# xiph/vorbis

Hardware: NVIDIA H100
Metric: stereo_blocks_per_sec_mdct_psy (higher is better)
Workload: dtype f32

## Files before the change

vorbis_b200/csrc/vb200.cu:

```cuda
#include <cuda_runtime.h>
#include <algorithm>
#include <atomic>
#include <cstdio>
#include <cstdlib>
#include <cstring>
#include <mutex>
#include <string>
#include <type_traits>
#include <vector>

#include "vorbis_b200.h"
#include "vb200_tables.h"
#include "vb200_kernels.cuh"
#include "vb200_cqn.cuh"
#include "vb200_psy2.cuh"
#include "vb200_psy3.cuh"
#include "vb200_floor1.cuh"
#include "vb200_env.cuh"
#include "vb200_res.cuh"
#include "vb200_streams.cuh"
#include "vb200_managed.cuh"
#include "floor1_db_table.h"

using namespace vb200;
// ... 1115 lines not shown
      case 1024: LAUNCH_XF(1024); break;
      case 2048: LAUNCH_XF(2048); break;
      default: LAUNCH_XF(0); break;
    }
#undef LAUNCH_XF
    rc = post_launch(c); if (rc) return rc;
  }
  return 0;
}

static int phaseA_psy_launch(vb200_ctx *c, int W, int nblocks, const vb200_phaseA_io *io, cudaStream_t st,
                             float *d_logfft, float *d_lmax, float *d_gmax) {
  const XformDev &X = c->dx[W];
  const int ch = c->setup.channels, N = X.N;
  const int rows = nblocks * ch;
  int rc;
  {
    const PsyDev &P0 = c->dpsy[2 * W], &P1 = c->dpsy[2 * W + 1];
    const size_t smem = psy2_smem(P0, P1);
    int rc = set_smem(k_phaseA_psy, smem); if (rc) return rc;
    {
      int &tuned = c->psy_carveout_ctas;
      const char *e = getenv("VB200_PSY_CTAS");
      const int ctas = e ? atoi(e) : c->psy_ctas_per_sm;
      if (tuned != ctas) {
        int pct = (int)((ctas * (smem + 1024) * 100 + 228 * 1024 - 1) / (228 * 1024));
        if (pct > 100) pct = 100;
        CU(cudaFuncSetAttribute(k_phaseA_psy, cudaFuncAttributePreferredSharedMemoryCarveout, pct));
        tuned = ctas;
      }
      c->psy_ctas_per_sm = ctas;
    }
    PhaseA2Args A;
    A.mdct_in = io->tap_mdct_raw ? io->tap_mdct_raw : io->mdct;
    A.logfft = d_logfft; A.lmax = d_lmax; A.gmax = d_gmax; A.desc = io->desc;
    A.mdct_out = io->mdct; A.logmdct = io->logmdct; A.logmask = io->logmask; A.ampmax_out = io->ampmax_out;
    A.tap_noise = io->tap_noise; A.tap_tone = io->tap_tone;
    { const char *e = getenv("VB200_DEBUG_SKIP"); A.dbg_skip = e ? atoi(e) : 0; }
    A.dbg_cycles = nullptr;
    if (getenv("VB200_PHASE_TIMING")) {
      void *p; if ((rc = ensure(c, 10, 16 * sizeof(unsigned long long), &p))) return rc;
      A.dbg_cycles = (unsigned long long *)p;
    }
    const int n = N / 2;
    const char *ev = getenv("VB200_PSY_V1");
    const bool v2ok = !(ev && atoi(ev)) && (n == 128 || n == 256 || n == 512 || n == 1024 || n == 2048);
    const char *ev2 = getenv("VB200_PSY_V2");
    const bool v3ok = v2ok && !(ev2 && atoi(ev2)) && P0.linesper == P1.linesper &&
                      psy3_supported(n, P0.total > P1.total ? P0.total : P1.total, P0.linesper);
    if (v3ok) {
      const int total = P0.total > P1.total ? P0.total : P1.total;
      const int nruns = P0.nruns > P1.nruns ? P0.nruns : P1.nruns;
      const int ngrp = P0.ngrp > P1.ngrp ? P0.ngrp : P1.ngrp;
      int R = 1;
      { const char *e = getenv("VB200_PSY_ROWS"); if (e) R = atoi(e) == 1 ? 1 : 2; }
      const size_t row_bytes = sizeof(float) * ((psy3_floats(n, total, nruns, ngrp) + 3) & ~(size_t)3);
      const size_t smem3 = row_bytes * R;
      int ctas = (int)((227 * 1024) / (smem3 + 1024));
      if (ctas > PSY3_MINB / R) ctas = PSY3_MINB / R;
      if (ctas < 1) ctas = 1;
      { const char *e = getenv("VB200_PSY_CTAS"); if (e) ctas = atoi(e); }
      const bool dbg3 = A.dbg_cycles || A.tap_noise || A.tap_tone;
#define LAUNCH_PSY3D(KK, RR, DD)                                                                   \
      do {                                                                                         \
        if ((rc = set_smem(k_phaseA_psy3<KK, RR, DD>, smem3))) return rc;                          \
        k_phaseA_psy3<KK, RR, DD><<<grid_for(c, (rows + RR - 1) / RR, ctas), PSY3_THREADS * RR, smem3, st>>>(P0, P1, ch, rows, A); \
      } while (0)
#define LAUNCH_PSY3R(KK, RR) do { if (dbg3) LAUNCH_PSY3D(KK, RR, true); else LAUNCH_PSY3D(KK, RR, false); } while (0)
#define LAUNCH_PSY4(KK)                                                                            \
      do {                                                                                         \
        if ((rc = set_smem(k_phaseA_psy4<KK>, row_bytes))) return rc;                              \
        k_phaseA_psy4<KK><<<grid_for(c, rows, PSY3_MINB), PSY3_THREADS, row_bytes, st>>>(P0, P1, ch, rows, A); \
      } while (0)
      static const bool psy_v4 = []() { const char *e = getenv("VB200_PSY_V4"); return e && atoi(e); }();
#define LAUNCH_PSY3(KK) do { if (psy_v4) LAUNCH_PSY4(KK); else if (R == 1) LAUNCH_PSY3R(KK, 1); else LAUNCH_PSY3R(KK, 2); } while (0)
      switch (n / 128) {
        case 1: LAUNCH_PSY3(1); break;
        case 2: LAUNCH_PSY3(2); break;
        case 4: LAUNCH_PSY3(4); break;
        case 8: LAUNCH_PSY3(8); break;
        default: LAUNCH_PSY3(16); break;
      }
#undef LAUNCH_PSY3R
#undef LAUNCH_PSY3D
#undef LAUNCH_PSY4
#undef LAUNCH_PSY3
    } else if (v2ok) {
      const int total = P0.total > P1.total ? P0.total : P1.total;
      const int nruns = P0.nruns > P1.nruns ? P0.nruns : P1.nruns;
      const int ngrp = P0.ngrp > P1.ngrp ? P0.ngrp : P1.ngrp;
      const size_t smem2 = sizeof(float) * psy2_floats(n, total, nruns, ngrp);
      int ctas = (int)((227 * 1024) / (smem2 + 1024));
      if (ctas > PSY2_MINB) ctas = PSY2_MINB;
      if (ctas < 1) ctas = 1;
      { const char *e = getenv("VB200_PSY_CTAS"); if (e) ctas = atoi(e); }
#define LAUNCH_PSY2(KK)                                                                            \
      do {                                                                                         \
        if ((rc = set_smem(k_phaseA_psy2<KK>, smem2))) return rc;                                  \
        k_phaseA_psy2<KK><<<grid_for(c, rows, ctas), PSY2_THREADS, smem2, st>>>(P0, P1, ch, rows, A); \
      } while (0)
      switch (n / 128) {
        case 1: LAUNCH_PSY2(1); break;
        case 2: LAUNCH_PSY2(2); break;
        case 4: LAUNCH_PSY2(4); break;
        case 8: LAUNCH_PSY2(8); break;
        default: LAUNCH_PSY2(16); break;
      }
#undef LAUNCH_PSY2
    } else {
      k_phaseA_psy<<<grid_for(c, rows, c->psy_ctas_per_sm), PSY_THREADS, smem, st>>>(P0, P1, ch, rows, A);
    }
    rc = post_launch(c); if (rc) return rc;
  }
  return 0;
}

static int phaseA_launch(vb200_ctx *c, int W, int nblocks, const vb200_phaseA_io *io,
                         int nstreams, int bps, const float *d_amp0, cudaStream_t st,
                         float *d_logfft, float *d_lmax, float *d_gmax, const PcmSrc *pcmsrc = nullptr) {
  PcmSrc psrc;
  if (pcmsrc) psrc = *pcmsrc;
  else { psrc.base = io->pcm; psrc.fmt = 0; psrc.bps = 1; psrc.hop = 0; psrc.stride = 0; psrc.blk_src = nullptr; }
  const XformDev &X = c->dx[W];
  const int ch = c->setup.channels, N = X.N;
  int rc;
  if (c->profiling) CU(cudaEventRecord(c->ev[0], st));
  if ((rc = phaseA_transform_launch(c, W, nblocks, io, psrc, st, d_logfft, d_lmax))) return rc;
  if (c->profiling) CU(cudaEventRecord(c->ev[1], st));
  {
    const int n = N / 2;
    const float secs = (float)n / (float)c->setup.rate;
    const float secs_att = secs * c->setup.ampmax_att_per_sec;
    if (nstreams > 0)
      k_ampmax<<<(nstreams + 127) / 128, 128, 0, st>>>(1, nstreams, bps, ch, io->desc, d_lmax, d_amp0, secs_att, d_gmax);
    else
      k_ampmax<<<(nblocks + 127) / 128, 128, 0, st>>>(0, nblocks, 0, ch, io->desc, d_lmax, nullptr, secs_att, d_gmax);
    int rc = post_launch(c); if (rc) return rc;
  }
// ... 1139 lines not shown
```

vorbis_b200/csrc/vb200_kernels.cuh:

```cuda
#pragma once
#include <cuda_runtime.h>
#include <stdint.h>
#include "vorbis_b200.h"

namespace vb200 {

#define VB_C1 .92387953251128675613F
#define VB_C2 .70710678118654752441F
#define VB_C3 .38268343236508977175F
#define VB_NEGINF (-9999.f)

struct XformDev {
  int N, log2n, nst, nf;
  int fac[8];
  int stage_off[8];
  float scale;
  const float  *trig;
  const int    *bitrev;
  const float2 *stage_tw;
  const float  *win;
  const float  *wa;
};

struct WinDev {
// ... 25 lines not shown
  const int *cls_off;
  int max_cls_len;
};

__device__ __forceinline__ float todB_dev(float x) {
  const unsigned int u = __float_as_uint(x) & 0x7fffffffu;
  return __uint2float_rn(u) * 7.17711438e-7f - 764.6161886f;
}
__device__ __forceinline__ float add345(float x) {
  return (float)((double)x + .345);
}

#ifndef VB200_EMU
__device__ __forceinline__ unsigned smem_u32(const void *p) { return (unsigned)__cvta_generic_to_shared(p); }
__device__ __forceinline__ float lds_f32(unsigned a) { float v; asm volatile("ld.shared.f32 %0, [%1];" : "=f"(v) : "r"(a)); return v; }
__device__ __forceinline__ int lds_s32(unsigned a) { int v; asm volatile("ld.shared.s32 %0, [%1];" : "=r"(v) : "r"(a)); return v; }
__device__ __forceinline__ int lds_s16(unsigned a) { short v; asm volatile("ld.shared.s16 %0, [%1];" : "=h"(v) : "r"(a)); return (int)v; }
__device__ __forceinline__ int4 lds_v4(unsigned a) { int4 v; asm volatile("ld.shared.v4.s32 {%0,%1,%2,%3}, [%4];" : "=r"(v.x), "=r"(v.y), "=r"(v.z), "=r"(v.w) : "r"(a)); return v; }
__device__ __forceinline__ float4 lds_f4(unsigned a) { float4 v; asm volatile("ld.shared.v4.f32 {%0,%1,%2,%3}, [%4];" : "=f"(v.x), "=f"(v.y), "=f"(v.z), "=f"(v.w) : "r"(a)); return v; }
__device__ __forceinline__ void sts_f4(unsigned a, float4 v) { asm volatile("st.shared.v4.f32 [%0], {%1,%2,%3,%4};" :: "r"(a), "f"(v.x), "f"(v.y), "f"(v.z), "f"(v.w) : "memory"); }
__device__ __forceinline__ void sts_s16(unsigned a, int v) { asm volatile("st.shared.s16 [%0], %1;" :: "r"(a), "h"((short)v) : "memory"); }
__device__ __forceinline__ void sts_f32(unsigned a, float v) { asm volatile("st.shared.f32 [%0], %1;" :: "r"(a), "f"(v) : "memory"); }
__device__ __forceinline__ void sts_s32(unsigned a, int v) { asm volatile("st.shared.s32 [%0], %1;" :: "r"(a), "r"(v) : "memory"); }
__device__ __forceinline__ void named_bar_sync(int barid, int nt) { asm volatile("bar.sync %0, %1;" :: "r"(barid), "r"(nt) : "memory"); }
__device__ __forceinline__ float lds_f32_if(unsigned a, float old, bool p) {
  asm volatile("{\n\t.reg .pred q;\n\tsetp.ne.b32 q, %2, 0;\n\t@q ld.shared.f32 %0, [%1];\n\t}" : "+f"(old) : "r"(a), "r"((int)p));
  return old;
}
__device__ __forceinline__ int lds_s16_if(unsigned a, int old, bool p) {
  short v = (short)old;
  asm volatile("{\n\t.reg .pred q;\n\tsetp.ne.b32 q, %2, 0;\n\t@q ld.shared.s16 %0, [%1];\n\t}" : "+h"(v) : "r"(a), "r"((int)p));
  return (int)v;
}
__device__ __forceinline__ int lds_s32_if(unsigned a, int old, bool p) {
  asm volatile("{\n\t.reg .pred q;\n\tsetp.ne.b32 q, %2, 0;\n\t@q ld.shared.s32 %0, [%1];\n\t}" : "+r"(old) : "r"(a), "r"((int)p));
  return old;
}
__device__ __forceinline__ void sts_s32_if(unsigned a, int v, bool p) {
  asm volatile("{\n\t.reg .pred q;\n\tsetp.ne.b32 q, %2, 0;\n\t@q st.shared.s32 [%0], %1;\n\t}" :: "r"(a), "r"(v), "r"((int)p) : "memory");
}
__device__ __forceinline__ void sts_f32_if(unsigned a, float v, bool p) {
  asm volatile("{\n\t.reg .pred q;\n\tsetp.ne.b32 q, %2, 0;\n\t@q st.shared.f32 [%0], %1;\n\t}" :: "r"(a), "f"(v), "r"((int)p) : "memory");
}
__device__ __forceinline__ void sts_s16_if(unsigned a, int v, bool p) {
  asm volatile("{\n\t.reg .pred q;\n\tsetp.ne.b32 q, %2, 0;\n\t@q st.shared.s16 [%0], %1;\n\t}" :: "r"(a), "h"((short)v), "r"((int)p) : "memory");
}
__device__ __forceinline__ void cp_async16(unsigned dst, const void *src) {
  asm volatile("cp.async.cg.shared.global [%0], [%1], 16;" :: "r"(dst), "l"(src) : "memory");
}
__device__ __forceinline__ void cp_async_commit() { asm volatile("cp.async.commit_group;" ::: "memory"); }
__device__ __forceinline__ void cp_async_wait_all() { asm volatile("cp.async.wait_group 0;" ::: "memory"); }
__device__ __forceinline__ void sts_release(unsigned a, int v) { asm volatile("st.release.cta.shared.s32 [%0], %1;" :: "r"(a), "r"(v) : "memory"); }
__device__ __forceinline__ int lds_acquire(unsigned a) { int v; asm volatile("ld.acquire.cta.shared.s32 %0, [%1];" : "=r"(v) : "r"(a) : "memory"); return v; }
__device__ __forceinline__ int lds_volatile(unsigned a) { int v; asm volatile("ld.volatile.shared.s32 %0, [%1];" : "=r"(v) : "r"(a) : "memory"); return v; }
__device__ __forceinline__ void fence_cta() { asm volatile("fence.acq_rel.cta;" ::: "memory"); }
__device__ __forceinline__ void spin_pause(unsigned ns) { __nanosleep(ns); }
__device__ __forceinline__ void prefetch_l2(const void *p) { asm volatile("prefetch.global.L2 [%0];" :: "l"(p)); }
__device__ __forceinline__ void mbar_init1(unsigned a) { asm volatile("mbarrier.init.shared::cta.b64 [%0], 1;" :: "r"(a) : "memory"); }
__device__ __forceinline__ void mbar_arrive_release(unsigned a) {
  asm volatile("{\n\t.reg .b64 st;\n\tmbarrier.arrive.relaxed.cta.shared::cta.b64 st, [%0];\n\t}" :: "r"(a) : "memory");
}
__device__ __forceinline__ void mbar_park(unsigned a, unsigned parity) {
  asm volatile("{\n\t.reg .pred p;\n\tmbarrier.try_wait.parity.acquire.cta.shared::cta.b64 p, [%0], %1;\n\t}" :: "r"(a), "r"(parity) : "memory");
}
#else
__device__ __forceinline__ unsigned smem_u32(const void *p) { return (unsigned)((const unsigned char *)p - cuemu::dyn_smem()); }
__device__ __forceinline__ float lds_f32(unsigned a) { return *reinterpret_cast<const float *>(cuemu::dyn_smem() + a); }
__device__ __forceinline__ int lds_s32(unsigned a) { return *reinterpret_cast<const int *>(cuemu::dyn_smem() + a); }
__device__ __forceinline__ int lds_s16(unsigned a) { return (int)*reinterpret_cast<const short *>(cuemu::dyn_smem() + a); }
__device__ __forceinline__ int4 lds_v4(unsigned a) { return *reinterpret_cast<const int4 *>(cuemu::dyn_smem() + a); }
__device__ __forceinline__ float4 lds_f4(unsigned a) { return *reinterpret_cast<const float4 *>(cuemu::dyn_smem() + a); }
__device__ __forceinline__ void sts_f4(unsigned a, float4 v) { *reinterpret_cast<float4 *>(cuemu::dyn_smem() + a) = v; }
__device__ __forceinline__ void sts_s16(unsigned a, int v) { *reinterpret_cast<short *>(cuemu::dyn_smem() + a) = (short)v; }
__device__ __forceinline__ void sts_f32(unsigned a, float v) { *reinterpret_cast<float *>(cuemu::dyn_smem() + a) = v; }
__device__ __forceinline__ void sts_s32(unsigned a, int v) { *reinterpret_cast<int *>(cuemu::dyn_smem() + a) = v; }
__device__ __forceinline__ void named_bar_sync(int barid, int nt) { cuemu_named_barrier(barid, nt); }
__device__ __forceinline__ void sts_release(unsigned a, int v) { __atomic_store_n(reinterpret_cast<int *>(cuemu::dyn_smem() + a), v, __ATOMIC_RELEASE); }
__device__ __forceinline__ int lds_acquire(unsigned a) { return __atomic_load_n(reinterpret_cast<int *>(cuemu::dyn_smem() + a), __ATOMIC_ACQUIRE); }
__device__ __forceinline__ int lds_volatile(unsigned a) { return __atomic_load_n(reinterpret_cast<int *>(cuemu::dyn_smem() + a), __ATOMIC_ACQUIRE); }
__device__ __forceinline__ void fence_cta() { __atomic_thread_fence(__ATOMIC_ACQ_REL); }
__device__ __forceinline__ void spin_pause(unsigned) { sched_yield(); }
__device__ __forceinline__ void prefetch_l2(const void *) {}
__device__ __forceinline__ void mbar_init1(unsigned) {}
__device__ __forceinline__ void mbar_arrive_release(unsigned) { __atomic_thread_fence(__ATOMIC_RELEASE); }
__device__ __forceinline__ void mbar_park(unsigned, unsigned) { sched_yield(); }
__device__ __forceinline__ void cp_async16(unsigned dst, const void *src) { memcpy(cuemu::dyn_smem() + dst, src, 16); }
__device__ __forceinline__ void cp_async_commit() {}
__device__ __forceinline__ void cp_async_wait_all() {}
__device__ __forceinline__ float lds_f32_if(unsigned a, float old, bool p) { return p ? lds_f32(a) : old; }
__device__ __forceinline__ int lds_s16_if(unsigned a, int old, bool p) { return p ? lds_s16(a) : old; }
__device__ __forceinline__ void sts_f32_if(unsigned a, float v, bool p) { if (p) sts_f32(a, v); }
__device__ __forceinline__ int lds_s32_if(unsigned a, int old, bool p) { return p ? lds_s32(a) : old; }
__device__ __forceinline__ void sts_s32_if(unsigned a, int v, bool p) { if (p) sts_s32(a, v); }
__device__ __forceinline__ void sts_s16_if(unsigned a, int v, bool p) { if (p) sts_s16(a, v); }
#endif

__device__ __forceinline__ float warp_max(float v) {
#pragma unroll
  for (int o = 16; o > 0; o >>= 1) v = fmaxf(v, __shfl_xor_sync(0xffffffffu, v, o));
  return v;
}


template <int NC> struct XLog2 { static constexpr int v = 1 + XLog2<NC / 2>::v; };
template <> struct XLog2<1> { static constexpr int v = 0; };
template <> struct XLog2<0> { static constexpr int v = 0; };

__device__ __forceinline__ int fly_pad(int a) { return a + 2 * (a >> 5) + 2 * (a >> 9); }

__device__ __forceinline__ void dev_fly8(const float4 v0, const float4 v1, float4 &o0, float4 &o1) {
  const float s62 = v1.z + v0.z, d62 = v1.z - v0.z;
  const float s40 = v1.x + v0.x, d40 = v1.x - v0.x;
  const float d51 = v1.y - v0.y, d73 = v1.w - v0.w;
  const float s51 = v1.y + v0.y, s73 = v1.w + v0.w;
  o1.z = s62 + s40;  o1.x = s62 - s40;
  o0.x = d62 + d51;  o0.z = d62 - d51;
  o0.w = d73 + d40;  o0.y = d73 - d40;
  o1.w = s73 + s51;  o1.y = s73 - s51;
}

template <int NC>
__device__ __forceinline__ void dev_butterflies(const XformDev &X, float *x, int tid, int nt, float *padbuf = nullptr) {
  const int N = NC ? NC : X.N;
  const int log2n = NC ? XLog2<NC>::v : X.log2n;
  const int nst = log2n - 6;
  const int n2 = N >> 1;
  const int items = n2 >> 2;
#pragma unroll
  for (int s = 0; s < nst; s++) {
    const int P = n2 >> s;
    const int lq = P >> 2;
    const int sh = log2n - 3 - s;
    const float2 *tw = X.stage_tw + X.stage_off[s];
    for (int u = tid; u < items; u += nt) {
      const int blk = u >> sh, q = u & (lq - 1);
      float *xb = x + P * blk;
      const int a = P - 2 - 2 * q, b = (P >> 1) - 2 - 2 * q;
      const float2 t = __ldg(tw + q);
// ... 808 lines not shown
```

vorbis_b200/csrc/vb200_psy3.cuh:

```cuda
#pragma once
#include "vb200_psy2.cuh"

namespace vb200 {

constexpr int PSY3_THREADS = 128;
constexpr int PSY3_L = 8;
constexpr int PSY3_RB = 7;
#ifndef PSY3_MINB
#define PSY3_MINB 8
#endif

__host__ __device__ inline bool psy3_supported(int n, int total, int linesper) {
  return linesper == PSY3_L && total <= PSY3_THREADS * PSY3_RB && total >= 2 * PSY3_L &&
         (n == 128 || n == 256 || n == 512 || n == 1024 || n == 2048);
}

__host__ __device__ inline size_t psy3_tone_floats(int n, int total, int nruns) {
  const int tp = (total + 7) & ~7, rp = (nruns + 3) & ~3;
  size_t a0 = 4 * (size_t)tp;
  if (a0 < (size_t)n) a0 = n;
  return a0 + 4 * (size_t)rp;
}
__host__ __device__ inline size_t psy3_floats(int n, int total, int nruns, int ngrp) {
  const size_t tone = psy3_tone_floats(n, total, nruns);
// ... 244 lines not shown
}

struct MixOut { float logmask, m, nz, tn; };
__device__ __noinline__ MixOut final_mix_val(float p2, float L, float p1, float noff, float ath, float gmin,
                                             const float *__restrict__ compand, MixConst C, float m) {
  MixOut o;
  const float work = L - p1;
  const float base = L - work;
  int dB = (int)((double)p2 + .5);
  if (dB >= VB200_COMPAND_LEVELS) dB = VB200_COMPAND_LEVELS - 1;
  if (dB < 0) dB = 0;
  const float nz = base + __ldg(compand + dB);
  float tn = ath + C.att;
  if (tn < gmin) tn = gmin;
  o.nz = nz; o.tn = tn;
  float val = nz + noff;
  if (val > C.noisemaxsupp) val = C.noisemaxsupp;
  const float t = tn + C.toneatt;
  o.logmask = val < t ? t : val;
  const float coeffi = -17.2f;
  float de;
  val = val - L;
  if (val > coeffi) {
    de = (float)(1.0 - ((double)(val - coeffi) * 0.005 * (double)C.m_val));
    if (de < 0.f) de = 0.0001f;
  } else {
    de = (float)(1.0 - ((double)(val - coeffi) * 0.0003 * (double)C.m_val));
  }
  o.m = m * de;
  return o;
}

template <int K, int R, bool DBG>
__global__ void __launch_bounds__(PSY3_THREADS * R, PSY3_MINB / R)
k_phaseA_psy3(PsyDev P0, PsyDev P1, int ch, int nrows, PhaseA2Args A) {
  extern __shared__ __align__(16) float sm_cta[];
  constexpr int nt = PSY3_THREADS;
  const int n = K * nt, ns = n + 4, tid = threadIdx.x & (nt - 1), half = threadIdx.x >> 7, lane = tid & 31;
  const int total = P0.total > P1.total ? P0.total : P1.total;
  const int nruns = P0.nruns > P1.nruns ? P0.nruns : P1.nruns;
  const int ngrp = P0.ngrp > P1.ngrp ? P0.ngrp : P1.ngrp;
  const int tp = (total + 7) & ~7;
  const size_t row_floats = (psy3_floats(n, total, nruns, ngrp) + 3) & ~(size_t)3;
  float *sm = sm_cta + half * row_floats;
  float *S = sm;
  float *s_fft = sm;
  float *copies = sm;
  size_t a0 = 4 * (size_t)tp; if (a0 < (size_t)n) a0 = n;
  int4 *run_rec = reinterpret_cast<int4 *>(sm + a0);
  const size_t area = psy3_floats(n, total, nruns, ngrp) - (size_t)((ngrp + 1 + 3) & ~3) - 16;
  float *grp_min = sm + area;
  int *s_misc = reinterpret_cast<int *>(grp_min + ((ngrp + 1 + 3) & ~3));
  for (int row0 = blockIdx.x * R; row0 < nrows; row0 += gridDim.x * R) {
    const int row = row0 + half < nrows ? row0 + half : nrows - 1;
    const int blk = row / ch;
    const PsyDev &P = A.desc[blk].blocktype ? P1 : P0;
    const float *gm = A.mdct_in + (size_t)row * n;
    const float *lf = A.logfft + (size_t)row * n;
    const float g = A.gmax[blk], lmax = A.lmax[row];
    const float att = tone_att(P, lmax);
    float L[K], M[K], p1[K];
    long long tmark = (DBG && A.dbg_cycles) ? clock64() : 0;
    int tph = 0;
#define PHASE_MARK()                                                              \
    do {                                                                          \
      if (DBG && A.dbg_cycles && threadIdx.x == 0) {                                     \
        const long long tnow = clock64();                                         \
        atomicAdd(A.dbg_cycles + tph, (unsigned long long)(tnow - tmark));        \
        tmark = tnow;                                                             \
      }                                                                           \
      tph++;                                                                      \
    } while (0)
#pragma unroll
    for (int k = 0; k < K; k++) {
      const int i = tid + k * nt;
      M[k] = __ldcs(gm + i);
      s_fft[i] = __ldcs(lf + i);
    }
#pragma unroll
    for (int k = 0; k < K; k++) {
      L[k] = add345(todB_dev(M[k]));
      __stcs(A.logmdct + (size_t)row * n + tid + k * nt, L[k]);
    }
#ifndef VB200_NO_PREFETCH
    {
      const int nrow = row0 + gridDim.x * R + half;
      if (nrow < nrows && tid < 2 * (n / 32)) {
        const float *src = tid < n / 32 ? A.mdct_in : A.logfft;
        prefetch_l2(src + (size_t)nrow * n + (tid & (n / 32 - 1)) * 32);
      }
    }
#endif
    __syncthreads();
    PHASE_MARK();
    dev_tone_runs3(P, s_fft, g, att, run_rec, tid);
    __syncthreads();
    PHASE_MARK();
    dev_tone_scatter3(P, copies, tp, run_rec, tid);
    __syncthreads();
    PHASE_MARK();
    dev_chase3<DBG>(P, copies, tp, s_misc, tid, half == 0 ? A.dbg_cycles : nullptr);
    PHASE_MARK();
    const float *seed = copies;
#pragma unroll 1
    for (int q = tid; q <= P.ngrp; q += nt) {
      float minV;
      if (q < P.ngrp) {
        const int4 gg = __ldg(P.grps + q);
        if (gg.y - gg.x > 16) continue;
        int pos = gg.x;
        minV = seed[pos];
        if (minV > P.tone_abs_limit) minV = P.tone_abs_limit;
#pragma unroll 1
        while (pos < gg.y) {
          pos++;
          const float s = seed[pos];
          if ((s > VB_NEGINF && s < minV) || minV == VB_NEGINF) minV = s;
        }
      } else {
        minV = seed[P.total - 1];
      }
      grp_min[q] = minV;
    }
#pragma unroll 1
    for (int li = tid >> 5; li < P.nlong; li += nt >> 5) {
      const int q = __ldg(P.long_grp + li);
      const int4 gg = __ldg(P.grps + q);
      float mn = 3.0e38f;
      int any = 0;
#pragma unroll 1
      for (int pos = gg.x + lane; pos <= gg.y; pos += 32) {
        const float s = seed[pos];
        if (s > VB_NEGINF) {
          any = 1;
          if (s < mn) mn = s;
          if (pos == gg.x && P.tone_abs_limit < mn) mn = P.tone_abs_limit;
        }
      }
#pragma unroll
      for (int o = 16; o > 0; o >>= 1) {
        mn = fminf(mn, __shfl_xor_sync(0xffffffffu, mn, o));
        any |= __shfl_xor_sync(0xffffffffu, any, o);
      }
      if (lane == 0) grp_min[q] = any ? mn : VB_NEGINF;
    }
    __syncthreads();
    PHASE_MARK();
    const int *bark = P.bark;
    const int bfe = P.bark_first_extra, ffe = P.fixed_first_extra, fixedw = P.noisewindowfixed;
    float p2[K];
#pragma unroll
    for (int k = 0; k < K; k++) p1[k] = 0.f;
#pragma unroll 1
    for (int pass = 0; pass < 2; pass++) {
      const float off = pass ? 0.f : 140.f;
      const int fx = pass ? fixedw : -1;
#pragma unroll
      for (int k = 0; k < K; k++) dev_noise_term1(tid + k * nt, L[k] - p1[k], off, S, ns);
      __syncthreads();
      PHASE_MARK();
      if (threadIdx.x < 5 * R) dev_noise_scan3(n, sm_cta + (threadIdx.x / 5) * row_floats + (threadIdx.x % 5) * ns);
      __syncthreads();
      PHASE_MARK();
      if (K >= 2) {
#pragma unroll
        for (int k = 0; k + 1 < K; k += 2) {
          const float2 r = regress_pair<K * PSY3_THREADS + 4>(bark, bfe, ffe, S, tid + k * nt, tid + (k + 1) * nt, off, fx);
          p2[k] = r.x; p2[k + 1] = r.y;
        }
      } else {
#pragma unroll
        for (int k = 0; k < K; k++) p2[k] = regress_core<K * PSY3_THREADS + 4>(bark, bfe, ffe, S, tid + k * nt, off, fx);
      }
      if (pass == 0) {
#pragma unroll
        for (int k = 0; k < K; k++) p1[k] = p2[k];
        __syncthreads();
        PHASE_MARK();
      }
    }
    MixConst MC;
    MC.noisemaxsupp = P.noisemaxsupp; MC.toneatt = P.tone_masteratt[1]; MC.m_val = P.m_val;
    MC.att = att;
    const float *noff = P.noiseoffset + n;
    const float *athp = P.ath, *compand = P.noisecompand;
    const short *bin_grp = P.bin_grp;
#pragma unroll
    for (int k = 0; k < K; k++) {
      const int i = tid + k * nt;
      const MixOut o = final_mix_val(p2[k], L[k], p1[k], __ldg(noff + i), __ldg(athp + i),
                                     grp_min[__ldg(bin_grp + i)], compand, MC, M[k]);
      __stcs(A.logmask + (size_t)row * n + i, o.logmask);
      __stcs(A.mdct_out + (size_t)row * n + i, o.m);
      if (DBG && A.tap_noise) A.tap_noise[(size_t)row * n + i] = o.nz;
      if (DBG && A.tap_tone) A.tap_tone[(size_t)row * n + i] = o.tn;
    }
    if (tid == 0 && (row % ch) == 0) A.ampmax_out[blk] = g;
    __syncthreads();
    PHASE_MARK();
#undef PHASE_MARK
  }
}

__device__ __forceinline__ void dev_noise_scan4(int n, float *S, int ns, int lane, unsigned a_prog, unsigned a_bar) {
  float4 *a = reinterpret_cast<float4 *>(S + (lane < 5 ? lane : 0) * ns);
  const int q = n >> 2;
  const bool act = lane < 5;
  float t = 0.f;
  float4 v0, v1, v2, v3, w0, w1, w2, w3;
  if (act) { v0 = a[0]; v1 = a[1]; v2 = a[2]; v3 = a[3]; }
#define SCAN4(v) do { t += v.x; v.x = t; t += v.y; v.y = t; t += v.z; v.z = t; t += v.w; v.w = t; } while (0)
  for (int i = 0; i < q; i += 8) {
    if (act) {
      w0 = a[i + 4]; w1 = a[i + 5]; w2 = a[i + 6]; w3 = a[i + 7];
      SCAN4(v0); SCAN4(v1); SCAN4(v2); SCAN4(v3);
      a[i] = v0; a[i + 1] = v1; a[i + 2] = v2; a[i + 3] = v3;
      if (i + 8 < q) { v0 = a[i + 8]; v1 = a[i + 9]; v2 = a[i + 10]; v3 = a[i + 11]; }
      SCAN4(w0); SCAN4(w1); SCAN4(w2); SCAN4(w3);
      a[i + 4] = w0; a[i + 5] = w1; a[i + 6] = w2; a[i + 7] = w3;
    }
    if ((i & 8) || i + 8 >= q) {
      __syncwarp();
      if (lane == 0) { sts_s32(a_prog, (i + 8) * 4); mbar_arrive_release(a_bar); }
    }
  }
#undef SCAN4
}

__device__ __forceinline__ void wait_progress(unsigned a_prog, unsigned a_bar, int need, int n, unsigned phase0) {
  need = __reduce_max_sync(0xffffffffu, need);
  if (need > n) need = n;
  for (int spins = 0; spins < (1 << 16); spins++) {
    const int p = lds_volatile(a_prog);
    if (p >= need) break;
    mbar_park(a_bar, (phase0 + ((unsigned)p >> 6)) & 1u);
  }
  fence_cta();
}

__device__ __forceinline__ void dev_final_mix(float p2, float L, float p1, float noff, float ath, float gmin,
                                              const float *__restrict__ compand, const MixConst &C, float m,
                                              float &logmask, float &m_out, float &nz_out, float &tn_out) {
  const float work = L - p1;
  const float base = L - work;
  int dB = (int)((double)p2 + .5);
  if (dB >= VB200_COMPAND_LEVELS) dB = VB200_COMPAND_LEVELS - 1;
  if (dB < 0) dB = 0;
  const float nz = base + __ldg(compand + dB);
  float tn = ath + C.att;
  if (tn < gmin) tn = gmin;
  nz_out = nz; tn_out = tn;
  float val = nz + noff;
  if (val > C.noisemaxsupp) val = C.noisemaxsupp;
  const float t = tn + C.toneatt;
  logmask = val < t ? t : val;
  const float coeffi = -17.2f;
  float de;
  val = val - L;
  if (val > coeffi) {
    de = (float)(1.0 - ((double)(val - coeffi) * 0.005 * (double)C.m_val));
    if (de < 0.f) de = 0.0001f;
  } else {
    de = (float)(1.0 - ((double)(val - coeffi) * 0.0003 * (double)C.m_val));
  }
  m_out = m * de;
}

template <int K>
__global__ void __launch_bounds__(PSY3_THREADS, PSY3_MINB)
k_phaseA_psy4(PsyDev P0, PsyDev P1, int ch, int nrows, PhaseA2Args A) {
  extern __shared__ __align__(16) float sm[];
  constexpr int nt = PSY3_THREADS;
  constexpr int NS = K * PSY3_THREADS + 4;
  const int n = K * nt, ns = n + 4, tid = threadIdx.x, lane = tid & 31;
  const int total = P0.total > P1.total ? P0.total : P1.total;
  const int nruns = P0.nruns > P1.nruns ? P0.nruns : P1.nruns;
  const int ngrp = P0.ngrp > P1.ngrp ? P0.ngrp : P1.ngrp;
  const int tp = (total + 7) & ~7;
  float *S = sm;
  float *s_fft = sm;
  float *copies = sm;
  size_t a0 = 4 * (size_t)tp; if (a0 < (size_t)n) a0 = n;
  int4 *run_rec = reinterpret_cast<int4 *>(sm + a0);
  const size_t area = psy3_floats(n, total, nruns, ngrp) - (size_t)((ngrp + 1 + 3) & ~3) - 16;
  float *grp_min = sm + area;
  int *s_misc = reinterpret_cast<int *>(grp_min + ((ngrp + 1 + 3) & ~3));
  const unsigned a_prog1 = smem_u32(s_misc + 8), a_prog2 = smem_u32(s_misc + 10);
  const unsigned a_bar1 = smem_u32(s_misc + 12), a_bar2 = smem_u32(s_misc + 14);
  if (tid == 0) { mbar_init1(a_bar1); mbar_init1(a_bar2); }
  __syncthreads();
  unsigned phase0 = 0;
  for (int row = blockIdx.x; row < nrows; row += gridDim.x, phase0 += (unsigned)(n >> 6)) {
    const int blk = row / ch;
    const PsyDev &P = A.desc[blk].blocktype ? P1 : P0;
    const float *gm = A.mdct_in + (size_t)row * n;
    const float *lf = A.logfft + (size_t)row * n;
    float *g_logmdct = A.logmdct + (size_t)row * n;
    float *g_logmask = A.logmask + (size_t)row * n;
    const float g = A.gmax[blk], lmax = A.lmax[row];
    const float att = tone_att(P, lmax);
    long long tmark = A.dbg_cycles ? clock64() : 0;
    int tph = 0;
#define PHASE_MARK()                                                              \
    do {                                                                          \
      if (A.dbg_cycles && tid == 0) {                                             \
        const long long tnow = clock64();                                         \
        atomicAdd(A.dbg_cycles + tph, (unsigned long long)(tnow - tmark));        \
        tmark = tnow;                                                             \
      }                                                                           \
      tph++;                                                                      \
    } while (0)
    if (tid < 4) s_misc[8 + tid] = 0;
#pragma unroll
    for (int k = 0; k < K; k++) {
      const int i = tid + k * nt;
      s_fft[i] = __ldcs(lf + i);
      __stcg(g_logmdct + i, add345(todB_dev(__ldcg(gm + i))));
    }
    __syncthreads();
    PHASE_MARK();
    dev_tone_runs3(P, s_fft, g, att, run_rec, tid);
    __syncthreads();
    PHASE_MARK();
    dev_tone_scatter3(P, copies, tp, run_rec, tid);
    __syncthreads();
    PHASE_MARK();
    dev_chase3<true>(P, copies, tp, s_misc, tid, A.dbg_cycles);
    PHASE_MARK();
    const float *seed = copies;
    for (int q = tid; q <= P.ngrp; q += nt) {
      float minV;
      if (q < P.ngrp) {
        const int4 gg = __ldg(P.grps + q);
        if (gg.y - gg.x > 16) continue;
        int pos = gg.x;
        minV = seed[pos];
        if (minV > P.tone_abs_limit) minV = P.tone_abs_limit;
        while (pos < gg.y) {
          pos++;
          const float s = seed[pos];
          if ((s > VB_NEGINF && s < minV) || minV == VB_NEGINF) minV = s;
        }
      } else {
        minV = seed[P.total - 1];
      }
      grp_min[q] = minV;
    }
    for (int li = tid >> 5; li < P.nlong; li += nt >> 5) {
      const int q = __ldg(P.long_grp + li);
      const int4 gg = __ldg(P.grps + q);
      float mn = 3.0e38f;
      int any = 0;
      for (int pos = gg.x + lane; pos <= gg.y; pos += 32) {
        const float s = seed[pos];
        if (s > VB_NEGINF) {
          any = 1;
          if (s < mn) mn = s;
          if (pos == gg.x && P.tone_abs_limit < mn) mn = P.tone_abs_limit;
        }
      }
#pragma unroll
      for (int o = 16; o > 0; o >>= 1) {
        mn = fminf(mn, __shfl_xor_sync(0xffffffffu, mn, o));
        any |= __shfl_xor_sync(0xffffffffu, any, o);
      }
      if (lane == 0) grp_min[q] = any ? mn : VB_NEGINF;
    }
    __syncthreads();
    PHASE_MARK();
    const int *bark = P.bark;
    const int bfe = P.bark_first_extra, ffe = P.fixed_first_extra, fixedw = P.noisewindowfixed;
    const int nchunks = n >> 5;
#pragma unroll
    for (int k = 0; k < K; k++) dev_noise_term1(tid + k * nt, __ldcg(g_logmdct + tid + k * nt), 140.f, S, ns);
    __syncthreads();
    PHASE_MARK();
    if (tid < 32) dev_noise_scan4(n, S, ns, lane, a_prog1, a_bar1);
    for (;;) {
      int c = 0;
      if (lane == 0) c = atomicAdd(s_misc + 9, 1);
      c = __shfl_sync(0xffffffffu, c, 0);
      if (c >= nchunks) break;
      const int i = c * 32 + lane;
      int need = 0;
      if (bfe > 0) { const int bk = __ldg(bark + (i < bfe ? i : bfe - 1)); need = (bk & 0xffff) + 1; }
      wait_progress(a_prog1, a_bar1, need, n, phase0);
      __stcg(g_logmask + i, dev_regress_bin<NS>(bark, bfe, ffe, S, i, 140.f, -1));
    }
    __syncthreads();
    PHASE_MARK();
    PHASE_MARK();
#pragma unroll
    for (int k = 0; k < K; k++)
      dev_noise_term1(tid + k * nt, __ldcg(g_logmdct + tid + k * nt) - __ldcg(g_logmask + tid + k * nt), 0.f, S, ns);
    __syncthreads();
    PHASE_MARK();
    MixConst MC;
    MC.noisemaxsupp = P.noisemaxsupp; MC.toneatt = P.tone_masteratt[1]; MC.m_val = P.m_val;
    MC.att = att;
    const float *noff = P.noiseoffset + n;
    const float *athp = P.ath, *compand = P.noisecompand;
    const short *bin_grp = P.bin_grp;
    if (tid < 32) dev_noise_scan4(n, S, ns, lane, a_prog2, a_bar2);
    for (;;) {
      int c = 0;
      if (lane == 0) c = atomicAdd(s_misc + 11, 1);
      c = __shfl_sync(0xffffffffu, c, 0);
      if (c >= nchunks) break;
      const int i = c * 32 + lane;
      int need = 0;
      if (bfe > 0) { const int bk = __ldg(bark + (i < bfe ? i : bfe - 1)); need = (bk & 0xffff) + 1; }
      if (fixedw > 0 && ffe > 0) { const int h2 = (i < ffe ? i : ffe - 1) + fixedw / 2 + 1; need = h2 > need ? h2 : need; }
      const float Lv = __ldcg(g_logmdct + i), p1v = __ldcg(g_logmask + i), mv = __ldcg(gm + i);
      const float nf = __ldg(noff + i), at = __ldg(athp + i), gmn = grp_min[__ldg(bin_grp + i)];
      wait_progress(a_prog2, a_bar2, need, n, phase0);
      const float p2 = dev_regress_bin<NS>(bark, bfe, ffe, S, i, 0.f, fixedw);
      float lm, mo, nz, tn;
      dev_final_mix(p2, Lv, p1v, nf, at, gmn, compand, MC, mv, lm, mo, nz, tn);
      __stcs(g_logmask + i, lm);
      __stcs(A.mdct_out + (size_t)row * n + i, mo);
      if (A.tap_noise) A.tap_noise[(size_t)row * n + i] = nz;
      if (A.tap_tone) A.tap_tone[(size_t)row * n + i] = tn;
    }
    if (tid == 0 && (row % ch) == 0) A.ampmax_out[blk] = g;
    __syncthreads();
    PHASE_MARK();
    PHASE_MARK();
#undef PHASE_MARK
  }
}

}
```

Before: 5.458 million.

## Default psy3 to two rows per CTA, drop M register array, remove psy4

The psy3 launch now always uses two rows per CTA (it previously defaulted to one), which doubles threads per block and halves the grid. The kernel no longer keeps the raw MDCT values in a register array; it reloads them from global memory in the final mix, cutting register pressure. Spare rows in the last pair skip the final stores. The experimental psy4 kernel and its mbarrier helpers are deleted. The reload adds memory traffic, and fixing R=2 changes occupancy and shared-memory use per CTA.

```diff
diff --git a/vorbis_b200/csrc/vb200.cu b/vorbis_b200/csrc/vb200.cu
--- a/vorbis_b200/csrc/vb200.cu
+++ b/vorbis_b200/csrc/vb200.cu
@@ -1191,8 +1191,7 @@
       const int total = P0.total > P1.total ? P0.total : P1.total;
       const int nruns = P0.nruns > P1.nruns ? P0.nruns : P1.nruns;
       const int ngrp = P0.ngrp > P1.ngrp ? P0.ngrp : P1.ngrp;
-      int R = 1;
-      { const char *e = getenv("VB200_PSY_ROWS"); if (e) R = atoi(e) == 1 ? 1 : 2; }
+      constexpr int R = 2;
       const size_t row_bytes = sizeof(float) * ((psy3_floats(n, total, nruns, ngrp) + 3) & ~(size_t)3);
       const size_t smem3 = row_bytes * R;
       int ctas = (int)((227 * 1024) / (smem3 + 1024));
@@ -1200,19 +1199,12 @@
       if (ctas < 1) ctas = 1;
       { const char *e = getenv("VB200_PSY_CTAS"); if (e) ctas = atoi(e); }
       const bool dbg3 = A.dbg_cycles || A.tap_noise || A.tap_tone;
-#define LAUNCH_PSY3D(KK, RR, DD)                                                                   \
+#define LAUNCH_PSY3D(KK, DD)                                                                       \
       do {                                                                                         \
-        if ((rc = set_smem(k_phaseA_psy3<KK, RR, DD>, smem3))) return rc;                          \
-        k_phaseA_psy3<KK, RR, DD><<<grid_for(c, (rows + RR - 1) / RR, ctas), PSY3_THREADS * RR, smem3, st>>>(P0, P1, ch, rows, A); \
+        if ((rc = set_smem(k_phaseA_psy3<KK, R, DD>, smem3))) return rc;                           \
+        k_phaseA_psy3<KK, R, DD><<<grid_for(c, (rows + R - 1) / R, ctas), PSY3_THREADS * R, smem3, st>>>(P0, P1, ch, rows, A); \
       } while (0)
-#define LAUNCH_PSY3R(KK, RR) do { if (dbg3) LAUNCH_PSY3D(KK, RR, true); else LAUNCH_PSY3D(KK, RR, false); } while (0)
-#define LAUNCH_PSY4(KK)                                                                            \
-      do {                                                                                         \
-        if ((rc = set_smem(k_phaseA_psy4<KK>, row_bytes))) return rc;                              \
-        k_phaseA_psy4<KK><<<grid_for(c, rows, PSY3_MINB), PSY3_THREADS, row_bytes, st>>>(P0, P1, ch, rows, A); \
-      } while (0)
-      static const bool psy_v4 = []() { const char *e = getenv("VB200_PSY_V4"); return e && atoi(e); }();
-#define LAUNCH_PSY3(KK) do { if (psy_v4) LAUNCH_PSY4(KK); else if (R == 1) LAUNCH_PSY3R(KK, 1); else LAUNCH_PSY3R(KK, 2); } while (0)
+#define LAUNCH_PSY3(KK) do { if (dbg3) LAUNCH_PSY3D(KK, true); else LAUNCH_PSY3D(KK, false); } while (0)
       switch (n / 128) {
         case 1: LAUNCH_PSY3(1); break;
         case 2: LAUNCH_PSY3(2); break;
@@ -1220,9 +1212,7 @@
         case 8: LAUNCH_PSY3(8); break;
         default: LAUNCH_PSY3(16); break;
       }
-#undef LAUNCH_PSY3R
 #undef LAUNCH_PSY3D
-#undef LAUNCH_PSY4
 #undef LAUNCH_PSY3
     } else if (v2ok) {
       const int total = P0.total > P1.total ? P0.total : P1.total;
diff --git a/vorbis_b200/csrc/vb200_kernels.cuh b/vorbis_b200/csrc/vb200_kernels.cuh
--- a/vorbis_b200/csrc/vb200_kernels.cuh
+++ b/vorbis_b200/csrc/vb200_kernels.cuh
@@ -101,17 +101,8 @@
 __device__ __forceinline__ void cp_async_wait_all() { asm volatile("cp.async.wait_group 0;" ::: "memory"); }
 __device__ __forceinline__ void sts_release(unsigned a, int v) { asm volatile("st.release.cta.shared.s32 [%0], %1;" :: "r"(a), "r"(v) : "memory"); }
 __device__ __forceinline__ int lds_acquire(unsigned a) { int v; asm volatile("ld.acquire.cta.shared.s32 %0, [%1];" : "=r"(v) : "r"(a) : "memory"); return v; }
-__device__ __forceinline__ int lds_volatile(unsigned a) { int v; asm volatile("ld.volatile.shared.s32 %0, [%1];" : "=r"(v) : "r"(a) : "memory"); return v; }
-__device__ __forceinline__ void fence_cta() { asm volatile("fence.acq_rel.cta;" ::: "memory"); }
 __device__ __forceinline__ void spin_pause(unsigned ns) { __nanosleep(ns); }
 __device__ __forceinline__ void prefetch_l2(const void *p) { asm volatile("prefetch.global.L2 [%0];" :: "l"(p)); }
-__device__ __forceinline__ void mbar_init1(unsigned a) { asm volatile("mbarrier.init.shared::cta.b64 [%0], 1;" :: "r"(a) : "memory"); }
-__device__ __forceinline__ void mbar_arrive_release(unsigned a) {
-  asm volatile("{\n\t.reg .b64 st;\n\tmbarrier.arrive.relaxed.cta.shared::cta.b64 st, [%0];\n\t}" :: "r"(a) : "memory");
-}
-__device__ __forceinline__ void mbar_park(unsigned a, unsigned parity) {
-  asm volatile("{\n\t.reg .pred p;\n\tmbarrier.try_wait.parity.acquire.cta.shared::cta.b64 p, [%0], %1;\n\t}" :: "r"(a), "r"(parity) : "memory");
-}
 #else
 __device__ __forceinline__ unsigned smem_u32(const void *p) { return (unsigned)((const unsigned char *)p - cuemu::dyn_smem()); }
 __device__ __forceinline__ float lds_f32(unsigned a) { return *reinterpret_cast<const float *>(cuemu::dyn_smem() + a); }
@@ -126,13 +117,8 @@
 __device__ __forceinline__ void named_bar_sync(int barid, int nt) { cuemu_named_barrier(barid, nt); }
 __device__ __forceinline__ void sts_release(unsigned a, int v) { __atomic_store_n(reinterpret_cast<int *>(cuemu::dyn_smem() + a), v, __ATOMIC_RELEASE); }
 __device__ __forceinline__ int lds_acquire(unsigned a) { return __atomic_load_n(reinterpret_cast<int *>(cuemu::dyn_smem() + a), __ATOMIC_ACQUIRE); }
-__device__ __forceinline__ int lds_volatile(unsigned a) { return __atomic_load_n(reinterpret_cast<int *>(cuemu::dyn_smem() + a), __ATOMIC_ACQUIRE); }
-__device__ __forceinline__ void fence_cta() { __atomic_thread_fence(__ATOMIC_ACQ_REL); }
 __device__ __forceinline__ void spin_pause(unsigned) { sched_yield(); }
 __device__ __forceinline__ void prefetch_l2(const void *) {}
-__device__ __forceinline__ void mbar_init1(unsigned) {}
-__device__ __forceinline__ void mbar_arrive_release(unsigned) { __atomic_thread_fence(__ATOMIC_RELEASE); }
-__device__ __forceinline__ void mbar_park(unsigned, unsigned) { sched_yield(); }
 __device__ __forceinline__ void cp_async16(unsigned dst, const void *src) { memcpy(cuemu::dyn_smem() + dst, src, 16); }
 __device__ __forceinline__ void cp_async_commit() {}
 __device__ __forceinline__ void cp_async_wait_all() {}
diff --git a/vorbis_b200/csrc/vb200_psy3.cuh b/vorbis_b200/csrc/vb200_psy3.cuh
--- a/vorbis_b200/csrc/vb200_psy3.cuh
+++ b/vorbis_b200/csrc/vb200_psy3.cuh
@@ -320,14 +320,15 @@
   float *grp_min = sm + area;
   int *s_misc = reinterpret_cast<int *>(grp_min + ((ngrp + 1 + 3) & ~3));
   for (int row0 = blockIdx.x * R; row0 < nrows; row0 += gridDim.x * R) {
-    const int row = row0 + half < nrows ? row0 + half : nrows - 1;
+    const bool spare = row0 + half >= nrows;
+    const int row = spare ? nrows - 1 : row0 + half;
     const int blk = row / ch;
     const PsyDev &P = A.desc[blk].blocktype ? P1 : P0;
     const float *gm = A.mdct_in + (size_t)row * n;
     const float *lf = A.logfft + (size_t)row * n;
     const float g = A.gmax[blk], lmax = A.lmax[row];
     const float att = tone_att(P, lmax);
-    float L[K], M[K], p1[K];
+    float L[K], p1[K];
     long long tmark = (DBG && A.dbg_cycles) ? clock64() : 0;
     int tph = 0;
 #define PHASE_MARK()                                                              \
@@ -342,12 +343,12 @@
 #pragma unroll
     for (int k = 0; k < K; k++) {
       const int i = tid + k * nt;
-      M[k] = __ldcs(gm + i);
+      L[k] = __ldcg(gm + i);
       s_fft[i] = __ldcs(lf + i);
     }
 #pragma unroll
     for (int k = 0; k < K; k++) {
-      L[k] = add345(todB_dev(M[k]));
+      L[k] = add345(todB_dev(L[k]));
       __stcs(A.logmdct + (size_t)row * n + tid + k * nt, L[k]);
     }
 #ifndef VB200_NO_PREFETCH
@@ -454,10 +455,10 @@
     const float *athp = P.ath, *compand = P.noisecompand;
     const short *bin_grp = P.bin_grp;
 #pragma unroll
-    for (int k = 0; k < K; k++) {
+    for (int k = 0; k < K && !spare; k++) {
       const int i = tid + k * nt;
       const MixOut o = final_mix_val(p2[k], L[k], p1[k], __ldg(noff + i), __ldg(athp + i),
-                                     grp_min[__ldg(bin_grp + i)], compand, MC, M[k]);
+                                     grp_min[__ldg(bin_grp + i)], compand, MC, __ldcs(gm + i));
       __stcs(A.logmask + (size_t)row * n + i, o.logmask);
       __stcs(A.mdct_out + (size_t)row * n + i, o.m);
       if (DBG && A.tap_noise) A.tap_noise[(size_t)row * n + i] = o.nz;
@@ -470,232 +471,4 @@
   }
 }
 
-__device__ __forceinline__ void dev_noise_scan4(int n, float *S, int ns, int lane, unsigned a_prog, unsigned a_bar) {
-  float4 *a = reinterpret_cast<float4 *>(S + (lane < 5 ? lane : 0) * ns);
-  const int q = n >> 2;
-  const bool act = lane < 5;
-  float t = 0.f;
-  float4 v0, v1, v2, v3, w0, w1, w2, w3;
-  if (act) { v0 = a[0]; v1 = a[1]; v2 = a[2]; v3 = a[3]; }
-#define SCAN4(v) do { t += v.x; v.x = t; t += v.y; v.y = t; t += v.z; v.z = t; t += v.w; v.w = t; } while (0)
-  for (int i = 0; i < q; i += 8) {
-    if (act) {
-      w0 = a[i + 4]; w1 = a[i + 5]; w2 = a[i + 6]; w3 = a[i + 7];
-      SCAN4(v0); SCAN4(v1); SCAN4(v2); SCAN4(v3);
-      a[i] = v0; a[i + 1] = v1; a[i + 2] = v2; a[i + 3] = v3;
-      if (i + 8 < q) { v0 = a[i + 8]; v1 = a[i + 9]; v2 = a[i + 10]; v3 = a[i + 11]; }
-      SCAN4(w0); SCAN4(w1); SCAN4(w2); SCAN4(w3);
-      a[i + 4] = w0; a[i + 5] = w1; a[i + 6] = w2; a[i + 7] = w3;
-    }
-    if ((i & 8) || i + 8 >= q) {
-      __syncwarp();
-      if (lane == 0) { sts_s32(a_prog, (i + 8) * 4); mbar_arrive_release(a_bar); }
-    }
-  }
-#undef SCAN4
-}
-
-__device__ __forceinline__ void wait_progress(unsigned a_prog, unsigned a_bar, int need, int n, unsigned phase0) {
-  need = __reduce_max_sync(0xffffffffu, need);
-  if (need > n) need = n;
-  for (int spins = 0; spins < (1 << 16); spins++) {
-    const int p = lds_volatile(a_prog);
-    if (p >= need) break;
-    mbar_park(a_bar, (phase0 + ((unsigned)p >> 6)) & 1u);
-  }
-  fence_cta();
-}
-
-__device__ __forceinline__ void dev_final_mix(float p2, float L, float p1, float noff, float ath, float gmin,
-                                              const float *__restrict__ compand, const MixConst &C, float m,
-                                              float &logmask, float &m_out, float &nz_out, float &tn_out) {
-  const float work = L - p1;
-  const float base = L - work;
-  int dB = (int)((double)p2 + .5);
-  if (dB >= VB200_COMPAND_LEVELS) dB = VB200_COMPAND_LEVELS - 1;
-  if (dB < 0) dB = 0;
-  const float nz = base + __ldg(compand + dB);
-  float tn = ath + C.att;
-  if (tn < gmin) tn = gmin;
-  nz_out = nz; tn_out = tn;
-  float val = nz + noff;
-  if (val > C.noisemaxsupp) val = C.noisemaxsupp;
-  const float t = tn + C.toneatt;
-  logmask = val < t ? t : val;
-  const float coeffi = -17.2f;
-  float de;
-  val = val - L;
-  if (val > coeffi) {
-    de = (float)(1.0 - ((double)(val - coeffi) * 0.005 * (double)C.m_val));
-    if (de < 0.f) de = 0.0001f;
-  } else {
-    de = (float)(1.0 - ((double)(val - coeffi) * 0.0003 * (double)C.m_val));
-  }
-  m_out = m * de;
-}
-
-template <int K>
-__global__ void __launch_bounds__(PSY3_THREADS, PSY3_MINB)
-k_phaseA_psy4(PsyDev P0, PsyDev P1, int ch, int nrows, PhaseA2Args A) {
-  extern __shared__ __align__(16) float sm[];
-  constexpr int nt = PSY3_THREADS;
-  constexpr int NS = K * PSY3_THREADS + 4;
-  const int n = K * nt, ns = n + 4, tid = threadIdx.x, lane = tid & 31;
-  const int total = P0.total > P1.total ? P0.total : P1.total;
-  const int nruns = P0.nruns > P1.nruns ? P0.nruns : P1.nruns;
-  const int ngrp = P0.ngrp > P1.ngrp ? P0.ngrp : P1.ngrp;
-  const int tp = (total + 7) & ~7;
-  float *S = sm;
-  float *s_fft = sm;
-  float *copies = sm;
-  size_t a0 = 4 * (size_t)tp; if (a0 < (size_t)n) a0 = n;
-  int4 *run_rec = reinterpret_cast<int4 *>(sm + a0);
-  const size_t area = psy3_floats(n, total, nruns, ngrp) - (size_t)((ngrp + 1 + 3) & ~3) - 16;
-  float *grp_min = sm + area;
-  int *s_misc = reinterpret_cast<int *>(grp_min + ((ngrp + 1 + 3) & ~3));
-  const unsigned a_prog1 = smem_u32(s_misc + 8), a_prog2 = smem_u32(s_misc + 10);
-  const unsigned a_bar1 = smem_u32(s_misc + 12), a_bar2 = smem_u32(s_misc + 14);
-  if (tid == 0) { mbar_init1(a_bar1); mbar_init1(a_bar2); }
-  __syncthreads();
-  unsigned phase0 = 0;
-  for (int row = blockIdx.x; row < nrows; row += gridDim.x, phase0 += (unsigned)(n >> 6)) {
-    const int blk = row / ch;
-    const PsyDev &P = A.desc[blk].blocktype ? P1 : P0;
-    const float *gm = A.mdct_in + (size_t)row * n;
-    const float *lf = A.logfft + (size_t)row * n;
-    float *g_logmdct = A.logmdct + (size_t)row * n;
-    float *g_logmask = A.logmask + (size_t)row * n;
-    const float g = A.gmax[blk], lmax = A.lmax[row];
-    const float att = tone_att(P, lmax);
-    long long tmark = A.dbg_cycles ? clock64() : 0;
-    int tph = 0;
-#define PHASE_MARK()                                                              \
-    do {                                                                          \
-      if (A.dbg_cycles && tid == 0) {                                             \
-        const long long tnow = clock64();                                         \
-        atomicAdd(A.dbg_cycles + tph, (unsigned long long)(tnow - tmark));        \
-        tmark = tnow;                                                             \
-      }                                                                           \
-      tph++;                                                                      \
-    } while (0)
-    if (tid < 4) s_misc[8 + tid] = 0;
-#pragma unroll
-    for (int k = 0; k < K; k++) {
-      const int i = tid + k * nt;
-      s_fft[i] = __ldcs(lf + i);
-      __stcg(g_logmdct + i, add345(todB_dev(__ldcg(gm + i))));
-    }
-    __syncthreads();
-    PHASE_MARK();
-    dev_tone_runs3(P, s_fft, g, att, run_rec, tid);
-    __syncthreads();
-    PHASE_MARK();
-    dev_tone_scatter3(P, copies, tp, run_rec, tid);
-    __syncthreads();
-    PHASE_MARK();
-    dev_chase3<true>(P, copies, tp, s_misc, tid, A.dbg_cycles);
-    PHASE_MARK();
-    const float *seed = copies;
-    for (int q = tid; q <= P.ngrp; q += nt) {
-      float minV;
-      if (q < P.ngrp) {
-        const int4 gg = __ldg(P.grps + q);
-        if (gg.y - gg.x > 16) continue;
-        int pos = gg.x;
-        minV = seed[pos];
-        if (minV > P.tone_abs_limit) minV = P.tone_abs_limit;
-        while (pos < gg.y) {
-          pos++;
-          const float s = seed[pos];
-          if ((s > VB_NEGINF && s < minV) || minV == VB_NEGINF) minV = s;
-        }
-      } else {
-        minV = seed[P.total - 1];
-      }
-      grp_min[q] = minV;
-    }
-    for (int li = tid >> 5; li < P.nlong; li += nt >> 5) {
-      const int q = __ldg(P.long_grp + li);
-      const int4 gg = __ldg(P.grps + q);
-      float mn = 3.0e38f;
-      int any = 0;
-      for (int pos = gg.x + lane; pos <= gg.y; pos += 32) {
-        const float s = seed[pos];
-        if (s > VB_NEGINF) {
-          any = 1;
-          if (s < mn) mn = s;
-          if (pos == gg.x && P.tone_abs_limit < mn) mn = P.tone_abs_limit;
-        }
-      }
-#pragma unroll
-      for (int o = 16; o > 0; o >>= 1) {
-        mn = fminf(mn, __shfl_xor_sync(0xffffffffu, mn, o));
-        any |= __shfl_xor_sync(0xffffffffu, any, o);
-      }
-      if (lane == 0) grp_min[q] = any ? mn : VB_NEGINF;
-    }
-    __syncthreads();
-    PHASE_MARK();
-    const int *bark = P.bark;
-    const int bfe = P.bark_first_extra, ffe = P.fixed_first_extra, fixedw = P.noisewindowfixed;
-    const int nchunks = n >> 5;
-#pragma unroll
-    for (int k = 0; k < K; k++) dev_noise_term1(tid + k * nt, __ldcg(g_logmdct + tid + k * nt), 140.f, S, ns);
-    __syncthreads();
-    PHASE_MARK();
-    if (tid < 32) dev_noise_scan4(n, S, ns, lane, a_prog1, a_bar1);
-    for (;;) {
-      int c = 0;
-      if (lane == 0) c = atomicAdd(s_misc + 9, 1);
-      c = __shfl_sync(0xffffffffu, c, 0);
-      if (c >= nchunks) break;
-      const int i = c * 32 + lane;
-      int need = 0;
-      if (bfe > 0) { const int bk = __ldg(bark + (i < bfe ? i : bfe - 1)); need = (bk & 0xffff) + 1; }
-      wait_progress(a_prog1, a_bar1, need, n, phase0);
-      __stcg(g_logmask + i, dev_regress_bin<NS>(bark, bfe, ffe, S, i, 140.f, -1));
-    }
-    __syncthreads();
-    PHASE_MARK();
-    PHASE_MARK();
-#pragma unroll
-    for (int k = 0; k < K; k++)
-      dev_noise_term1(tid + k * nt, __ldcg(g_logmdct + tid + k * nt) - __ldcg(g_logmask + tid + k * nt), 0.f, S, ns);
-    __syncthreads();
-    PHASE_MARK();
-    MixConst MC;
-    MC.noisemaxsupp = P.noisemaxsupp; MC.toneatt = P.tone_masteratt[1]; MC.m_val = P.m_val;
-    MC.att = att;
-    const float *noff = P.noiseoffset + n;
-    const float *athp = P.ath, *compand = P.noisecompand;
-    const short *bin_grp = P.bin_grp;
-    if (tid < 32) dev_noise_scan4(n, S, ns, lane, a_prog2, a_bar2);
-    for (;;) {
-      int c = 0;
-      if (lane == 0) c = atomicAdd(s_misc + 11, 1);
-      c = __shfl_sync(0xffffffffu, c, 0);
-      if (c >= nchunks) break;
-      const int i = c * 32 + lane;
-      int need = 0;
-      if (bfe > 0) { const int bk = __ldg(bark + (i < bfe ? i : bfe - 1)); need = (bk & 0xffff) + 1; }
-      if (fixedw > 0 && ffe > 0) { const int h2 = (i < ffe ? i : ffe - 1) + fixedw / 2 + 1; need = h2 > need ? h2 : need; }
-      const float Lv = __ldcg(g_logmdct + i), p1v = __ldcg(g_logmask + i), mv = __ldcg(gm + i);
-      const float nf = __ldg(noff + i), at = __ldg(athp + i), gmn = grp_min[__ldg(bin_grp + i)];
-      wait_progress(a_prog2, a_bar2, need, n, phase0);
-      const float p2 = dev_regress_bin<NS>(bark, bfe, ffe, S, i, 0.f, fixedw);
-      float lm, mo, nz, tn;
-      dev_final_mix(p2, Lv, p1v, nf, at, gmn, compand, MC, mv, lm, mo, nz, tn);
-      __stcs(g_logmask + i, lm);
-      __stcs(A.mdct_out + (size_t)row * n + i, mo);
-      if (A.tap_noise) A.tap_noise[(size_t)row * n + i] = nz;
-      if (A.tap_tone) A.tap_tone[(size_t)row * n + i] = tn;
-    }
-    if (tid == 0 && (row % ch) == 0) A.ampmax_out[blk] = g;
-    __syncthreads();
-    PHASE_MARK();
-    PHASE_MARK();
-#undef PHASE_MARK
-  }
-}
-
-}
+}
```

New measurement: 5.626 million, median of 6. 1.03x the previous value.
